# seceq/zkir

Hardware: AMD Instinct MI355X
Metric: trace rows/sec (2^20-cycle fib: execution-trace fill + BabyBear NTT/LDE + Poseidon2 Merkle commitment) (higher is better)
Workload: dtype u32 (Baby Bear, 31-bit modular) / u64 trace words

## Files before the change

### zkir_amd/csrc/host.h

```cpp
#pragma once

#include <sys/mman.h>

#include <atomic>
#include <cstdint>
#include <cstdlib>
#include <cstring>
#include <new>
#include <string>
#include <utility>
#include <vector>

#include "../../include/zkir_amd.h"

#define ZKIR_DEFAULT_TILE_ROWS 1024u

namespace zkir {

struct Status {
  int code = ZKIR_OK;
  std::string msg;
  bool ok() const { return code == ZKIR_OK; }
};

// ... 130 lines not shown
  void* d_block = nullptr;
  const uint32_t* d_tape = nullptr; const uint32_t* h_tape = nullptr;
  const uint64_t* d_side = nullptr;
  const uint64_t* d_prefix = nullptr;
  uint64_t n_words = 0, n_hcells = 0, n_calls = 0;
  HashWitness() = default;
  HashWitness(const HashWitness&) = delete;
  HashWitness& operator=(const HashWitness&) = delete;
  ~HashWitness();
};
int memcheck_device_hash(const zkir_trace_columns* trace, uint64_t n_real, const uint8_t* blob, size_t blob_len, const zkir_hash_out* outs, uint64_t n_outs, uint64_t* mem_old,
                         uint32_t* mem_told, std::vector<uint64_t>& cell_addr, std::vector<uint64_t>& cell_bytes, std::vector<uint32_t>& cell_time, HashWitness& hw, HostPin& pin,
                         void* hip_stream);

struct LdeTables {
  int log_n;
  const uint32_t* tw_inv;
  const uint32_t* tw_fwd;
  const uint32_t* g_lo;
  const uint32_t* g_hi;
  const uint32_t* small_inv;
  const uint32_t* small_fwd;
  int log_blowup = 1;
};
void lde_run(const LdeTables& t, uint32_t* in, uint32_t n_blocks, uint32_t* out, void* hip_stream);
bool strided_variant_run(const LdeTables& t, uint32_t* data, uint32_t n_blocks, int variant, bool dit, void* hip_stream);
bool lde_run_fused01(const LdeTables& t, const zkir_trace_columns* trace, uint64_t n_real, uint32_t* in, uint32_t n_blocks, uint32_t* out, void* hip_stream);
}
```

### zkir_amd/csrc/ntt.hip

```cpp
#include <hip/hip_runtime.h>

#include <atomic>
#include <cstdlib>
#include <mutex>
#include <type_traits>

#include "../../include/zkir_amd.h"
#include "../../include/zkir_amd_experimental.h"
#include "babybear.h"
#include "host.h"

namespace {

constexpr int NT = 256;
__device__ __forceinline__ uint32_t bitrev(uint32_t x, int bits) { return bits == 0 ? 0u : __brev(x) >> (32 - bits); }

template <int K, int N, class F>
__device__ __forceinline__ void static_for(F&& f) {
  if constexpr (K < N) { f(std::integral_constant<int, K>{}); static_for<K + 1, N>(f); }
}

using u32x4 = uint32_t __attribute__((ext_vector_type(4)));
__device__ __forceinline__ u32x4 ld4(const uint4* p) { return *reinterpret_cast<const u32x4*>(p); }
__device__ __forceinline__ void st4(uint4* p, u32x4 v) { *reinterpret_cast<u32x4*>(p) = v; }
// ... 52 lines not shown
  if (blk == 0 && half == 0) {
    const uint64_t pcv = q.t.pc[src];
    r.x = (uint32_t)((q.t.cycle[src] + (i - src)) % bb::P); r.y = (uint32_t)(pcv & 0xFFFFF); r.z = (uint32_t)((pcv >> 20) & 0xFFFFF); r.w = (uint32_t)(pcv >> 40);
  } else if (blk == 0) {
    const uint32_t w = q.t.instruction[src];
    r.x = w & 0x7F; r.y = (w >> 7) & 0xF; r.z = (w >> 11) & 0xF; r.w = (w >> 15) & 0xF;
  } else {
    auto limbs = [&](int g, uint32_t out[3]) {
      const uint64_t o = (uint64_t)g * q.t.reg_stride + src;
      const uint64_t v = q.t.registers[o];
      const int bits = q.t.reg_state[o] ? 30 : 20;
      const uint64_t mask = (1ull << bits) - 1;
      out[0] = (uint32_t)(v & mask); out[1] = (uint32_t)((v >> bits) & mask); out[2] = (uint32_t)(v >> (2 * bits));
    };
    uint32_t a[3], b[3];
    if (half == 0) { limbs(1, a); r.x = q.t.instruction[src] >> 19; r.y = a[0]; r.z = a[1]; r.w = a[2]; }
    else { limbs(2, a); limbs(3, b); r.x = a[0]; r.y = a[1]; r.z = a[2]; r.w = b[0]; }
  }
  return r;
}

template <bool DIT, int R, int C, int NTH, bool FUSED = false>
__global__ __launch_bounds__(NTH) void ntt_strided_r4_kernel(uint4* __restrict__ data, uint64_t blk_u4, uint32_t tiles_per_block, uint32_t total, int L, int s0,
                                                              const uint32_t* __restrict__ tw, const uint32_t* __restrict__ small, int log_small, uint32_t j4_m, int canon, TraceSrc01 fsrc = TraceSrc01{}) {
  constexpr int B = 2 * R;
  constexpr uint32_t POS = 1u << (B + C), QUADS = POS / 4, CMASK = (1u << C) - 1, PLANE = POS + 4;
  constexpr uint32_t MOVES = 2 * POS / NTH;
  static_assert(QUADS % NTH == 0 && NTH % (1 << C) == 0 && (2 * POS) % NTH == 0, "tile / thread geometry");
  extern __shared__ uint4 lds4[];
  const uint32_t n = 1u << L;
  const uint32_t stride_mid = DIT ? (1u << s0) : (n >> (s0 + B));
  const uint32_t lo_tiles = stride_mid >> C;
  auto geometry = [&](uint32_t w, uint4*& x, uint32_t& base, uint32_t& lo0, uint32_t& hi) {
    const uint32_t tile = w % tiles_per_block;
    x = data + (uint64_t)(w / tiles_per_block) * blk_u4;
    hi = tile / lo_tiles;
    lo0 = (tile % lo_tiles) << C;
    base = (DIT ? (hi << (s0 + B)) : hi * (n >> s0)) + lo0;
  };
  static_assert(QUADS == NTH, "one quad per lane and round");
  u32x4 pre[MOVES];
  uint4* x; uint32_t base, lo0, hi;
  uint32_t w = blockIdx.x;
  if (w >= total) return;
  uint32_t sm[R];
#pragma unroll
  for (int r = 0; r < R; r++) {
    const int b = 2 * r;
    const uint32_t qq = threadIdx.x >> C;
    if (!DIT) sm[r] = small[bitrev(qq >> (B - 2 - b), b) << (log_small - (b + 2))];
    else sm[r] = small[(qq & ((1u << b) - 1)) << (log_small - (b + 2))];
  }
  const bool unit = s0 == 0;
  uint32_t tf_next[R] = {};
  auto tile_factors = [&](uint32_t hi_t) {
    if (DIT || unit) return;
    const uint32_t e = bitrev(hi_t, s0);
#pragma unroll
    for (int r = 0; r < R; r++) tf_next[r] = tw[e << (L - s0 - 2 * r - 2)];
  };
  geometry(w, x, base, lo0, hi);
  static_for<0, (int)MOVES>([&](auto kc) {
    constexpr uint32_t k = decltype(kc)::value;
    const uint32_t e = threadIdx.x + k * NTH, row = e >> (C + 1), wv = e & ((2u << C) - 1);
    if constexpr (FUSED) pre[k] = trace_quad01(fsrc, w / tiles_per_block, wv & 1, (uint64_t)base + (uint64_t)row * stride_mid + (wv >> 1));
    else pre[k] = ld4(&x[((uint64_t)base + (uint64_t)row * stride_mid) * 2 + wv]);
  });
  uint32_t tw_cur = 0;
  if (DIT) tw_cur = tw[(lo0 + (threadIdx.x & CMASK)) << (L - s0 - B)];
  tile_factors(hi);
  for (;;) {
    static_for<0, (int)MOVES>([&](auto kc) {
      constexpr uint32_t k = decltype(kc)::value;
      const uint32_t e = threadIdx.x + k * NTH, row = e >> (C + 1), wv = e & ((2u << C) - 1);
      st4(&lds4[(wv & 1) * PLANE + ((row << C) | (wv >> 1))], pre[k]);
    });
    uint32_t tp[R];
    if (DIT) {
      uint32_t u = tw_cur;
#pragma unroll
      for (int r = R - 1; r >= 0; r--) { tp[r] = u; u = bb::mont_mul(u, u); u = bb::mont_mul(u, u); }
    } else {
#pragma unroll
      for (int r = 0; r < R; r++) tp[r] = tf_next[r];
    }
    __syncthreads();
    const uint32_t wn = w + gridDim.x;
    uint4* xn = x; uint32_t base_n = base, lo0_n = lo0, hi_n = hi;
    if (wn < total) {
      geometry(wn, xn, base_n, lo0_n, hi_n);
      static_for<0, (int)MOVES>([&](auto kc) {
        constexpr uint32_t k = decltype(kc)::value;
        const uint32_t e = threadIdx.x + k * NTH, row = e >> (C + 1), wv = e & ((2u << C) - 1);
        if constexpr (FUSED) pre[k] = trace_quad01(fsrc, wn / tiles_per_block, wv & 1, (uint64_t)base_n + (uint64_t)row * stride_mid + (wv >> 1));
        else pre[k] = ld4(&xn[((uint64_t)base_n + (uint64_t)row * stride_mid) * 2 + wv]);
      });
      if (DIT) tw_cur = tw[(lo0_n + (threadIdx.x & CMASK)) << (L - s0 - B)];
      tile_factors(hi_n);
    }
#pragma unroll
    for (int r = 0; r < R; r++) {
      const int b = 2 * r;
#pragma unroll
      for (uint32_t k = 0; k < QUADS / NTH; k++) {
        uint32_t q = threadIdx.x + k * NTH;
        asm volatile("" : "+v"(q));
        const uint32_t lo_l = q & CMASK, qq = q >> C;
        uint4* pl0 = lds4; uint4* pl1 = lds4 + PLANE;
        if constexpr (!DIT) {
          const int lg = B - 2 - b;
          const uint32_t h2 = 1u << lg, mid_lo = qq & (h2 - 1), mid_hi = qq >> lg;
          const uint32_t i0 = ((((mid_hi << (lg + 2)) | mid_lo)) << C) | lo_l, d = h2 << C;
          WTw w1, w2, w2i;
          ct_twiddles(sm[r], tp[r], unit, j4_m, w1, w2, w2i);
          uint4 x0 = pl0[i0], x1 = pl0[i0 + d], x2 = pl0[i0 + 2 * d], x3 = pl0[i0 + 3 * d];
          ct4w4(x0, x1, x2, x3, w1, w2, w2i);
          pl0[i0] = x0; pl0[i0 + d] = x1; pl0[i0 + 2 * d] = x2; pl0[i0 + 3 * d] = x3;
          __builtin_amdgcn_sched_barrier(0);
          uint4 y0 = pl1[i0], y1 = pl1[i0 + d], y2 = pl1[i0 + 2 * d], y3 = pl1[i0 + 3 * d];
          ct4w4(y0, y1, y2, y3, w1, w2, w2i);
          pl1[i0] = y0; pl1[i0 + d] = y1; pl1[i0 + 2 * d] = y2; pl1[i0 + 3 * d] = y3;
        } else {
// ... 1 lines not shown
          const uint32_t i0 = ((((mid_hi << (b + 2)) | mid_lo)) << C) | lo_l, d = dm << C;
          const WTw w2 = wtw(bb::mont_mul_centred(tp[r], sm[r]));
          const uint32_t w2u = bb::wcanon(w2.w);
          const WTw w1 = wtw(bb::mont_mul_centred(w2u, w2u)), w2i = wtw(bb::mont_mul_centred(w2u, j4_m));
          uint4 x0 = pl0[i0], x1 = pl0[i0 + d], x2 = pl0[i0 + 2 * d], x3 = pl0[i0 + 3 * d];
          dit4w4(x0, x1, x2, x3, w1, w2, w2i);
          pl0[i0] = x0; pl0[i0 + d] = x1; pl0[i0 + 2 * d] = x2; pl0[i0 + 3 * d] = x3;
          __builtin_amdgcn_sched_barrier(0);
          uint4 y0 = pl1[i0], y1 = pl1[i0 + d], y2 = pl1[i0 + 2 * d], y3 = pl1[i0 + 3 * d];
          dit4w4(y0, y1, y2, y3, w1, w2, w2i);
          pl1[i0] = y0; pl1[i0 + d] = y1; pl1[i0 + 2 * d] = y2; pl1[i0 + 3 * d] = y3;
        }
      }
      const bool wave_local = !DIT ? (r + 1 < R && B - 2 - b <= 6 - C) : (r + 1 < R && b + 2 <= 6 - C);
      if (wave_local) wave_sync_lds(); else __syncthreads();
    }
#pragma unroll
    for (uint32_t k = 0; k < MOVES; k++) {
      const uint32_t e = threadIdx.x + k * NTH, row = e >> (C + 1), wv = e & ((2u << C) - 1);
      uint4 v = lds4[(wv & 1) * PLANE + ((row << C) | (wv >> 1))];
      if (DIT && canon) v = canon4(v);
      x[((uint64_t)base + (uint64_t)row * stride_mid) * 2 + wv] = v;
    }
    if (wn >= total) break;
    w = wn; x = xn; base = base_n; lo0 = lo0_n; hi = hi_n;
  }
}

template <bool DIT, int S>
__global__ __launch_bounds__(NT) void ntt_reg_kernel(uint4* __restrict__ data, uint64_t blk_u4, int L, int s0, const uint32_t* __restrict__ tw, uint32_t r4_m, uint32_t r8_m,
                                                       uint32_t r8_3_m, int canon) {
  constexpr int E = 1 << S;
  const uint32_t n = 1u << L;
  uint4* x = data + (uint64_t)blockIdx.y * blk_u4;
  const uint64_t item = (uint64_t)blockIdx.x * NT + threadIdx.x;
  if (item >= ((uint64_t)n >> S) * 2) return;
  const uint32_t t = (uint32_t)(item >> 1), h = (uint32_t)(item & 1);
  const uint32_t d = DIT ? (1u << s0) : (n >> (s0 + S));
  const uint32_t hi = t / d, lo = t % d;
  const uint64_t base = ((uint64_t)hi * d * E + lo) * 2 + h;
  uint4 v[E];
#pragma unroll
  for (int k = 0; k < E; k++) v[k] = x[base + (uint64_t)k * d * 2];
  if (!DIT) {
    const uint32_t Tf = tw[bitrev(hi, s0) << (L - s0 - S)];
    const uint32_t Tm = bb::mont_mul(Tf, Tf);
// ... 22 lines not shown
    }
    if (canon) {
#pragma unroll
      for (int k = 0; k < E; k++) v[k] = canon4(v[k]);
    }
  }
#pragma unroll
  for (int k = 0; k < E; k++) x[base + (uint64_t)k * d * 2] = v[k];
}

inline unsigned cu_count() {
  static std::mutex mu;
  static unsigned cached[64] = {};
  int dev = 0;
  if (hipGetDevice(&dev) != hipSuccess || dev < 0 || dev >= 64) return 256u;
  std::lock_guard<std::mutex> lk(mu);
  if (!cached[dev]) { hipDeviceProp_t p; cached[dev] = hipGetDeviceProperties(&p, dev) == hipSuccess && p.multiProcessorCount > 0 ? (unsigned)p.multiProcessorCount : 256u; }
  return cached[dev];
}
inline int persist() { static const int v = getenv("ZKIR_NTT_PERSIST") ? atoi(getenv("ZKIR_NTT_PERSIST")) : 1; return v; }

template <bool DIT, int R, int C, int NTH, bool FUSED = false>
void launch_strided_r4(uint32_t* data, uint64_t n, uint32_t n_blocks, int L, int s0, const uint32_t* tw, const uint32_t* small, int log_small, uint32_t j4_m, hipStream_t s,
                       const TraceSrc01* fsrc = nullptr, int canon = 0) {
  constexpr size_t lds = 16u * 2 * ((1u << (2 * R + C)) + 4);
  auto k = ntt_strided_r4_kernel<DIT, R, C, NTH, FUSED>;
  static std::atomic<uint64_t> attr_done{0};
  int dev = 0; (void)hipGetDevice(&dev);
  const uint64_t bit = 1ull << (dev & 63);
  if (!(attr_done.load(std::memory_order_relaxed) & bit)) { (void)hipFuncSetAttribute(reinterpret_cast<const void*>(k), hipFuncAttributeMaxDynamicSharedMemorySize, (int)lds); attr_done.fetch_or(bit); }
  const uint32_t tiles = (uint32_t)(n >> (2 * R + C)), total = tiles * n_blocks;
  const unsigned per_cu = (unsigned)((160u << 10) / lds) > 0 ? (unsigned)((160u << 10) / lds) : 1u;
  unsigned grid = persist() ? cu_count() * (per_cu > 8 ? 8 : per_cu) : total;
  if (grid > total) grid = total;
  hipLaunchKernelGGL(k, dim3(grid), dim3(NTH), lds, s, (uint4*)data, 2 * n, tiles, total, L, s0, tw, small, log_small, j4_m, canon, fsrc ? *fsrc : TraceSrc01{});
}

inline int strided_c() { static const int c = getenv("ZKIR_NTT_C") ? atoi(getenv("ZKIR_NTT_C")) : 2; return c; }

template <bool DIT>
void run_strided_stages(uint32_t* data, uint64_t n, uint32_t n_blocks, int L, int s0, int stages, const uint32_t* tw, const uint32_t* small, int log_small, uint32_t j4_m,
                        uint32_t r8_m, uint32_t r8_3_m, hipStream_t s) {
  while (stages > 0) {
    int take;
    if (stages >= 10 && stages != 11) take = 10;
    else if (stages == 11) take = 8;
    else if (stages == 9) take = 6;
    else if (stages == 7) take = 4;
    else if (stages == 5) take = 3;
    else take = stages;
    const int canon = DIT && take == stages;
    switch (take) {
      case 10:
        if (strided_c() == 2) launch_strided_r4<DIT, 5, 2, 1024>(data, n, n_blocks, L, s0, tw, small, log_small, j4_m, s, nullptr, canon);
        else launch_strided_r4<DIT, 5, 1, 512>(data, n, n_blocks, L, s0, tw, small, log_small, j4_m, s, nullptr, canon);
        break;
      case 8: launch_strided_r4<DIT, 4, 3, 512>(data, n, n_blocks, L, s0, tw, small, log_small, j4_m, s, nullptr, canon); break;
      case 6: launch_strided_r4<DIT, 3, 4, 256>(data, n, n_blocks, L, s0, tw, small, log_small, j4_m, s, nullptr, canon); break;
      case 4: launch_strided_r4<DIT, 2, 5, 128>(data, n, n_blocks, L, s0, tw, small, log_small, j4_m, s, nullptr, canon); break;
      case 3:
        hipLaunchKernelGGL((ntt_reg_kernel<DIT, 3>), dim3((unsigned)(((n >> 3) * 2 + NT - 1) / NT), n_blocks), dim3(NT), 0, s, (uint4*)data, 2 * n, L, s0, tw, j4_m, r8_m, r8_3_m, canon);
        break;
      case 2:
        hipLaunchKernelGGL((ntt_reg_kernel<DIT, 2>), dim3((unsigned)(((n >> 2) * 2 + NT - 1) / NT), n_blocks), dim3(NT), 0, s, (uint4*)data, 2 * n, L, s0, tw, j4_m, r8_m, r8_3_m, canon);
        break;
      default:
        hipLaunchKernelGGL(ntt_stage_kernel<DIT>, dim3((unsigned)((n + NT - 1) / NT), n_blocks), dim3(NT), 0, s, (uint4*)data, 2 * n, L, s0, tw, canon);
        break;
    }
    s0 += take; stages -= take;
  }
}

__global__ __launch_bounds__(NT) void lde_small_kernel(const uint32_t* __restrict__ in, uint32_t* __restrict__ out, int L, const uint32_t* __restrict__ small_inv,
                                                        const uint32_t* __restrict__ small_fwd, const uint32_t* __restrict__ g_lo, const uint32_t* __restrict__ g_hi) {
  extern __shared__ uint32_t lds[];
  const uint32_t n = 1u << L;
  const uint32_t* x = in + (uint64_t)blockIdx.x * n * 8;
  uint32_t* y = out + (uint64_t)blockIdx.x * 2 * n * 8;
  for (int c = 0; c < 8; c++) {
    for (uint32_t e = threadIdx.x; e < n; e += NT) lds[e] = x[(uint64_t)e * 8 + c];
    __syncthreads();
    for (int b = 0; b < L; b++) {
      const int hb = L - 1 - b;
      const uint32_t half = 1u << hb;
      for (uint32_t q = threadIdx.x; q < (n >> 1); q += NT) {
        const uint32_t r_lo = q & (half - 1), r_hi = q >> hb;
        const uint32_t ia = (r_hi << (hb + 1)) | r_lo, ib = ia + half;
        const uint32_t a = lds[ia], bv = lds[ib];
        lds[ia] = bb::add(a, bv); lds[ib] = bb::mont_mul(bb::sub(a, bv), small_inv[r_lo << b]);
      }
      __syncthreads();
    }
    uint32_t v[2];
// ... 1 lines not shown
    for (uint32_t e = threadIdx.x; e < n; e += NT) { const uint32_t k = bitrev(e, L); v[cnt++] = bb::mont_mul(bb::mont_mul(lds[e], g_lo[k & 1023]), g_hi[k >> 10]); }
    __syncthreads();
    cnt = 0;
    for (uint32_t e = threadIdx.x; e < n; e += NT) { lds[2 * e] = v[cnt]; lds[2 * e + 1] = v[cnt]; cnt++; }
    __syncthreads();
    for (int s = 1; s <= L; s++) {
      const uint32_t half = 1u << s;
      for (uint32_t q = threadIdx.x; q < n; q += NT) {
        const uint32_t r_lo = q & (half - 1), r_hi = q >> s;
        const uint32_t ia = (r_hi << (s + 1)) | r_lo, ib = ia + half;
        const uint32_t a = lds[ia], t = bb::mont_mul(lds[ib], small_fwd[r_lo << (L - s)]);
        lds[ia] = bb::add(a, t); lds[ib] = bb::sub(a, t);
      }
      __syncthreads();
    }
    for (uint32_t e = threadIdx.x; e < 2 * n; e += NT) y[(uint64_t)e * 8 + c] = lds[e];
    __syncthreads();
  }
}

constexpr int MID_NT = 512;
__global__ __launch_bounds__(MID_NT) __attribute__((amdgpu_waves_per_eu(4, 4))) void lde_middle_r4_kernel(const uint4* __restrict__ in, uint4* __restrict__ out, uint32_t chunks_per_block, uint32_t total, int L,
                                                                const uint32_t* __restrict__ tw_inv, const uint32_t* __restrict__ small_inv, const uint32_t* __restrict__ small_fwd,
                                                                const uint32_t* __restrict__ g_lo, const uint32_t* __restrict__ g_hi, uint32_t j4_inv_m, uint32_t j4_fwd_m, int canon) {
  constexpr int Bm = 10;
  constexpr uint32_t APL = 1024;
  __shared__ uint4 A[2 * APL];
  __shared__ uint4 Bf[2048];
  const uint32_t n = 1u << L, t = threadIdx.x;
  uint32_t w = blockIdx.x;
  if (w >= total) return;
  uint32_t tw_i[5], tw_f[5];
#pragma unroll
  for (int r = 0; r < 5; r++) {
    const int lg = 8 - 2 * r;
    tw_i[r] = small_inv[bitrev((t & 255) >> lg, 2 * r) << lg];
    const int sft = 2 * r + 1;
    tw_f[r] = small_fwd[(t & ((1u << sft) - 1)) << (Bm - sft - 1)];
  }
  u32x4 pre[4];
  uint32_t cf_next[5];
  uint32_t glo[4], ghi[4];
  auto fetch = [&](uint32_t ww) {
    const uint4* x = in + ((uint64_t)(ww / chunks_per_block) * n + ((uint64_t)(ww % chunks_per_block) << Bm)) * 2;
#pragma unroll
    for (int k = 0; k < 4; k++) pre[k] = ld4(&x[t + k * MID_NT]);
    const uint32_t p0 = ((ww % chunks_per_block) << Bm) + 4 * (t & 255);
#pragma unroll
    for (int i = 0; i < 4; i++) { const uint32_t k = bitrev(p0 + i, L); glo[i] = g_lo[k & 1023]; ghi[i] = g_hi[k >> 10]; }
    const uint32_t ce = bitrev(ww % chunks_per_block, L - Bm);
#pragma unroll
    for (int r = 0; r < 5; r++) cf_next[r] = tw_inv[ce << (8 - 2 * r)];
  };
  fetch(w);
  for (;;) {
    const uint32_t base = (w % chunks_per_block) << Bm;
    uint4* y = out + (uint64_t)(w / chunks_per_block) * n * 4;
#pragma unroll
    for (int k = 0; k < 4; k++) { const uint32_t e = t + k * MID_NT; st4(&A[(e & 1) * APL + (e >> 1)], pre[k]); }
    uint32_t gs[4];
#pragma unroll
    for (int i = 0; i < 4; i++) gs[i] = bb::mont_mul(glo[i], ghi[i]);
    uint32_t cf[5];
#pragma unroll
    for (int r = 0; r < 5; r++) cf[r] = cf_next[r];
    __syncthreads();
    const uint32_t wn = w + gridDim.x;
    if (wn < total) fetch(wn);
    {
      const uint32_t q = t & 255;
      uint4* a = A + (t >> 8) * APL;
#pragma unroll
      for (int r = 0; r < 5; r++) {
        const int lg = 8 - 2 * r;
        const uint32_t h2 = 1u << lg, lo = q & (h2 - 1), hi = q >> lg;
        const uint32_t i0 = (hi << (lg + 2)) | lo;
        WTw c1, c2, c2i;
        ct_twiddles(tw_i[r], cf[r], false, j4_inv_m, c1, c2, c2i);
        uint4 x0 = a[i0], x1 = a[i0 + h2], x2 = a[i0 + 2 * h2], x3 = a[i0 + 3 * h2];
        ct4w4(x0, x1, x2, x3, c1, c2, c2i);
        if (r == 4) {
          x0 = scale4(x0, gs[0]); x1 = scale4(x1, gs[1]); x2 = scale4(x2, gs[2]); x3 = scale4(x3, gs[3]);
        }
        a[i0] = x0; a[i0 + h2] = x1; a[i0 + 2 * h2] = x2; a[i0 + 3 * h2] = x3;
        if (r >= 1 && r < 4) wave_sync_lds(); else __syncthreads();
      }
    }
#pragma unroll 1
    for (int h = 0; h < 2; h++) {
      const uint4* a = A + h * APL;
// ... 183 lines not shown
  static const uint32_t j4_inv_m = bb::to_mont(bb::inv(bb::root_of_unity(2))), j4_fwd_m = bb::to_mont(bb::root_of_unity(2));
  static const uint32_t r8_fwd = bb::root_of_unity(3), r8_inv = bb::inv(r8_fwd);
  static const uint32_t r8_inv_m = bb::to_mont(r8_inv), r8_inv3_m = bb::to_mont(bb::mul(bb::mul(r8_inv, r8_inv), r8_inv));
  static const uint32_t r8_fwd_m = bb::to_mont(r8_fwd), r8_fwd3_m = bb::to_mont(bb::mul(bb::mul(r8_fwd, r8_fwd), r8_fwd));
  const int LB = t.log_blowup;
  if (LB != 1) {
    if (L < 10) {
      hipLaunchKernelGGL(lde_small_blowup_kernel, dim3(n_blocks), dim3(NT), (4u << (L + LB)), s, in, out, L, LB, t.small_inv, t.small_fwd, t.g_lo, t.g_hi);
      return;
    }
    run_strided_stages<false>(in, N, n_blocks, L, 0, L - 10, t.tw_inv, t.small_inv, 10, j4_inv_m, r8_inv_m, r8_inv3_m, s);
    const uint32_t chunks = N >> 10, total = chunks * n_blocks;
    unsigned grid = persist() ? cu_count() * 2 : total;
    if (grid > total) grid = total;
    auto mid = LB == 2 ? lde_middle_blowup_kernel<2> : lde_middle_blowup_kernel<3>;
    hipLaunchKernelGGL(mid, dim3(grid), dim3(MID_NT), 0, s, (const uint4*)in, (uint4*)out, chunks, total, L, t.tw_inv, t.small_inv, t.small_fwd, t.g_lo, t.g_hi, j4_inv_m, j4_fwd_m, L == 10);
    run_strided_stages<true>(out, (uint64_t)N << LB, n_blocks, L + LB, 10 + LB, L - 10, t.tw_fwd, t.small_fwd, 10 + LB, j4_fwd_m, r8_fwd_m, r8_fwd3_m, s);
    return;
  }
  if (L < 10) {
    hipLaunchKernelGGL(lde_small_kernel, dim3(n_blocks), dim3(NT), (8u << L), s, in, out, L, t.small_inv, t.small_fwd, t.g_lo, t.g_hi);
    return;
  }
  run_strided_stages<false>(in, N, n_blocks, L, 0, L - 10, t.tw_inv, t.small_inv, 10, j4_inv_m, r8_inv_m, r8_inv3_m, s);
  {
    const uint32_t chunks = N >> 10, total = chunks * n_blocks;
    unsigned grid = persist() ? cu_count() * 2 : total;
    if (grid > total) grid = total;
    hipLaunchKernelGGL(lde_middle_r4_kernel, dim3(grid), dim3(MID_NT), 0, s, (const uint4*)in, (uint4*)out, chunks, total, L, t.tw_inv, t.small_inv, t.small_fwd, t.g_lo, t.g_hi,
                       j4_inv_m, j4_fwd_m, L == 10);
  }
  run_strided_stages<true>(out, (uint64_t)2 * N, n_blocks, L + 1, 11, L - 10, t.tw_fwd, t.small_fwd, 11, j4_fwd_m, r8_fwd_m, r8_fwd3_m, s);
}


bool strided_variant_run(const LdeTables& t, uint32_t* data, uint32_t n_blocks, int variant, bool dit, void* stream) {
  hipStream_t s = (hipStream_t)stream;
  const int L = dit ? t.log_n + 1 : t.log_n;
  if (t.log_n < 20) return false;
  const uint64_t n = (uint64_t)1 << L;
  static const uint32_t j4_inv_m = bb::to_mont(bb::inv(bb::root_of_unity(2))), j4_fwd_m = bb::to_mont(bb::root_of_unity(2));
  const uint32_t* tw = dit ? t.tw_fwd : t.tw_inv; const uint32_t* sm = dit ? t.small_fwd : t.small_inv;
  const int ls = dit ? 11 : 10; const uint32_t j4 = dit ? j4_fwd_m : j4_inv_m; const int s0 = dit ? 11 : 0;
#define ZKIR_VARIANT(R, C, NTH) do { if (dit) launch_strided_r4<true, R, C, NTH>(data, n, n_blocks, L, s0, tw, sm, ls, j4, s); else launch_strided_r4<false, R, C, NTH>(data, n, n_blocks, L, s0, tw, sm, ls, j4, s); } while (0)
  switch (variant) {
    case 0: ZKIR_VARIANT(5, 2, 1024); break;
    case 1: ZKIR_VARIANT(5, 1, 512); break;
    case 2: ZKIR_VARIANT(4, 3, 512); break;
    case 3: ZKIR_VARIANT(4, 2, 256); break;
    case 4: ZKIR_VARIANT(3, 4, 256); break;
    default: return false;
  }
#undef ZKIR_VARIANT
  return true;
}

bool lde_run_fused01(const LdeTables& t, const zkir_trace_columns* trace, uint64_t n_real, uint32_t* in, uint32_t n_blocks, uint32_t* out, void* stream) {
  hipStream_t s = (hipStream_t)stream;
  const int L = t.log_n;
  if (L < 20 || L == 21 || n_blocks < 3 || strided_c() != 2) return false;
  const uint32_t N = 1u << L;
  static const uint32_t j4_inv_m = bb::to_mont(bb::inv(bb::root_of_unity(2))), j4_fwd_m = bb::to_mont(bb::root_of_unity(2));
  static const uint32_t r8_fwd = bb::root_of_unity(3), r8_inv = bb::inv(r8_fwd);
  static const uint32_t r8_inv_m = bb::to_mont(r8_inv), r8_inv3_m = bb::to_mont(bb::mul(bb::mul(r8_inv, r8_inv), r8_inv));
  static const uint32_t r8_fwd_m = bb::to_mont(r8_fwd), r8_fwd3_m = bb::to_mont(bb::mul(bb::mul(r8_fwd, r8_fwd), r8_fwd));
  const TraceSrc01 src{*trace, n_real};
  launch_strided_r4<false, 5, 2, 1024, true>(in, N, 2, L, 0, t.tw_inv, t.small_inv, 10, j4_inv_m, s, &src);
  launch_strided_r4<false, 5, 2, 1024>(in + (uint64_t)2 * N * 8, N, n_blocks - 2, L, 0, t.tw_inv, t.small_inv, 10, j4_inv_m, s);
  if (L - 10 > 10) run_strided_stages<false>(in, N, n_blocks, L, 10, L - 20, t.tw_inv, t.small_inv, 10, j4_inv_m, r8_inv_m, r8_inv3_m, s);
  {
    const uint32_t chunks = N >> 10, total = chunks * n_blocks;
    unsigned grid = persist() ? cu_count() * 2 : total;
    if (grid > total) grid = total;
    hipLaunchKernelGGL(lde_middle_r4_kernel, dim3(grid), dim3(MID_NT), 0, s, (const uint4*)in, (uint4*)out, chunks, total, L, t.tw_inv, t.small_inv, t.small_fwd, t.g_lo, t.g_hi,
                       j4_inv_m, j4_fwd_m, L == 10);
  }
  run_strided_stages<true>(out, (uint64_t)2 * N, n_blocks, L + 1, 11, L - 10, t.tw_fwd, t.small_fwd, 11, j4_fwd_m, r8_fwd_m, r8_fwd3_m, s);
  return true;
}

}
```

### zkir_amd/csrc/stark.hip

```cpp
#include <hip/hip_runtime.h>

#include <array>
#include <atomic>
#include <chrono>
#include <cstdio>
#include <cstdlib>
#include <cstddef>
#include <memory>
#include <mutex>
#include <vector>

#include "../../include/zkir_amd.h"
#include "../../include/zkir_amd_experimental.h"
#include "air.h"
#include "babybear.h"
#include "fri_shape.h"
#include "host.h"
#include "hashcall.h"
#include "poseidon2.h"
#include "verify_stages.h"

namespace {

constexpr int NT = 256;
// ... 577 lines not shown
}

__global__ __launch_bounds__(NT) void modmul_peak_kernel(uint32_t* __restrict__ out, uint32_t iters) {
  uint32_t a[8], c[8];
#pragma unroll
  for (int k = 0; k < 8; k++) { a[k] = (threadIdx.x * 2654435761u + blockIdx.x * 40503u + k * 7919u) % bb::P; c[k] = (a[k] * 31u + 7u) % bb::P; }
  for (uint32_t i = 0; i < iters; i++) {
#pragma unroll
    for (int k = 0; k < 8; k++) a[k] = bb::mont_mul_lazy(a[k], c[k]);
  }
  uint32_t r = 0;
#pragma unroll
  for (int k = 0; k < 8; k++) r ^= a[k];
  if (r == 0xFFFFFFFFu && iters == 0xFFFFFFFFu) out[0] = r;
}

constexpr uint32_t SYNC_SLOTS = 1024;
struct SyncRing {
  uint32_t* d_slots = nullptr;
  std::atomic<uint32_t> next{0};
  uint32_t* take() { return d_slots + (next.fetch_add(1, std::memory_order_relaxed) % SYNC_SLOTS); }
};

void launch_tree_levels(const p2::Consts* cp, uint32_t* leaf_digests, uint64_t n_leaves, SyncRing& ring, hipStream_t s) {
  uint32_t* cur = leaf_digests;
  uint64_t m = n_leaves;
  for (; m > (1u << 18); m >>= 1) {
    uint32_t* nxt = cur + 4 * m;
    hipLaunchKernelGGL(compress_kernel, dim3(grid_for(m / 2)), dim3(NT), 0, s, cp, cur, m / 2, nxt);
    cur = nxt;
  }
  if (m > 1) {
    const uint32_t per = m < SUBTREE ? (uint32_t)m : SUBTREE;
    hipLaunchKernelGGL(subtree_kernel, dim3((unsigned)(m / per)), dim3(NT_SUB), 0, s, cp, cur, m, per, ring.take());
  }
}

}

struct zkir_stark_ctx {
  uint32_t log_n = 0, log_blowup = 1;
  uint32_t* d_tw_inv = nullptr;
  uint32_t* d_tw_fwd = nullptr;
  uint32_t* d_g_lo = nullptr;
  uint32_t* d_g_lo_m = nullptr;
  mutable uint32_t* d_inv_xm1 = nullptr;
  uint32_t* d_g_hi = nullptr;
  uint32_t* d_small_inv = nullptr;
  uint32_t* d_small_fwd = nullptr;
  p2::Consts consts;
  p2::Consts* d_p2 = nullptr;
  mutable hipStream_t ov_stream = nullptr; mutable hipEvent_t ov_ev[2] = {nullptr, nullptr}; mutable std::vector<hipEvent_t> ov_group_ev; mutable uint4* d_ov_state = nullptr; mutable size_t ov_state_bytes = 0;
  mutable SyncRing sync;
  mutable std::mutex mu;
  mutable unsigned char* arena = nullptr;
  mutable size_t arena_size = 0, arena_off = 0;
  mutable zkir::HostPin pin;
  mutable const uint32_t* rate_mats[3] = {nullptr, nullptr, nullptr};
  mutable uint32_t rate_widths[3] = {0, 0, 0};
};

namespace {
const char* const BLOWUP2_ONLY = ": the context has log_blowup != 1; the prover's quotient, DEEP and FRI stages (and the experiments built on its LDE) are blow-up 2 — contexts of log_blowup 2 / 3 serve zkir_lde_launch and the zkir_merkle_* calls";
bool blowup2_only(const zkir_stark_ctx* c, const char* who) {
  if (c->log_blowup == 1) return true;
  zkir::set_last_error({ZKIR_ERR_ARGUMENT, std::string(who) + BLOWUP2_ONLY});
  return false;
}
int lde_launch(const zkir_stark_ctx* c, uint32_t* in, uint32_t width, uint32_t* out, bool mont_out, hipStream_t s) {
  const zkir::LdeTables t{(int)c->log_n, c->d_tw_inv, c->d_tw_fwd, mont_out ? c->d_g_lo_m : c->d_g_lo, c->d_g_hi, c->d_small_inv, c->d_small_fwd, (int)c->log_blowup};
  zkir::lde_run(t, in, (width + 7) / 8, out, s);
  return check_launch("lde");
}
int merkle_commit(const zkir_stark_ctx* c, const uint32_t* mat, uint32_t width, uint64_t n_leaves, uint32_t* tree, bool mont_in, hipStream_t s) {
  hipLaunchKernelGGL(leaf_hash_kernel, dim3(grid_for(n_leaves)), dim3(NT), 0, s, c->d_p2, mat, width, n_leaves, mont_in ? bb::from_mont(c->consts.in_scale) : c->consts.in_scale, tree);
  launch_tree_levels(c->d_p2, tree, n_leaves, c->sync, s);
  return check_launch("merkle_commit");
}
int selector_table_ensure(const zkir_stark_ctx* c, hipStream_t s) {
  if (c->d_inv_xm1) return ZKIR_OK;
  const uint64_t M = 1ull << (c->log_n + c->log_blowup);
  uint32_t* t = nullptr;
  if (hipMalloc(&t, (size_t)M * 4) != hipSuccess) { zkir::set_last_error({ZKIR_ERR_DEVICE, "zkir_prove_rate: no device memory for the selector table"}); return ZKIR_ERR_DEVICE; }
  hipLaunchKernelGGL(selector_inverse_kernel, dim3(grid_for((M + 7) / 8)), dim3(NT), 0, s, c->log_n + c->log_blowup, c->d_tw_fwd, t);
  c->d_inv_xm1 = t;
  return check_launch("selector table");
}
}

extern "C" {

uint32_t zkir_main_trace_width(void) { return air::committed_width(false); }
uint32_t zkir_main_trace_width_for(uint32_t deferred) { return air::committed_width((int)deferred); }
// ... 69 lines not shown
  (void)hipEventSynchronize(b);
  float ms = 0;
  (void)hipEventElapsedTime(&ms, a, b);
  (void)hipEventDestroy(a); (void)hipEventDestroy(b); (void)hipFree(d);
  return ms > 0 ? (double)blocks * NT * iters * 8.0 / (ms * 1e-3) : 0.0;
}

int zkir_stark_ctx_create(uint32_t log_n, uint32_t log_blowup, zkir_stark_ctx** out) {
  if (!out || log_n < 1 || log_n > 26 || log_blowup < 1 || log_blowup > 3 || log_n + log_blowup > 27) {
    zkir::set_last_error({ZKIR_ERR_ARGUMENT, "zkir_stark_ctx_create: need 1 <= log_n <= 26, log_blowup in {1, 2, 3} and log_n + log_blowup <= 27 (the field's two-adicity)"});
    return ZKIR_ERR_ARGUMENT;
  }
  *out = nullptr;
  zkir_stark_ctx* c = new zkir_stark_ctx();
  c->log_n = log_n; c->log_blowup = log_blowup;
  const uint32_t N = 1u << log_n;
  const uint32_t n_inv = N >= 2 ? N / 2 : 1, n_hi = (N >> 10) + 1;
  const uint32_t n_fwd = N << (log_blowup - 1);
  p2::generate(c->consts);
  hipError_t e = hipMalloc((void**)&c->d_p2, sizeof(p2::Consts));
  if (e == hipSuccess) e = hipMemcpy(c->d_p2, &c->consts, sizeof(p2::Consts), hipMemcpyHostToDevice);
  if (e == hipSuccess) e = hipMalloc(&c->sync.d_slots, SYNC_SLOTS * sizeof(uint32_t));
  if (e == hipSuccess) e = hipMemset(c->sync.d_slots, 0, SYNC_SLOTS * sizeof(uint32_t));
  if (e == hipSuccess) e = hipMalloc(&c->d_tw_inv, (size_t)n_inv * 4);
  if (e == hipSuccess) e = hipMalloc(&c->d_tw_fwd, (size_t)n_fwd * 4);
  if (e == hipSuccess) e = hipMalloc(&c->d_g_lo, 1024 * 4);
  if (e == hipSuccess) e = hipMalloc(&c->d_g_hi, (size_t)n_hi * 4);
  if (e == hipSuccess) e = hipMalloc(&c->d_g_lo_m, 1024 * 4);
  if (e == hipSuccess && log_blowup == 1) e = hipMalloc(&c->d_inv_xm1, (size_t)2 * N * 4);
  const int Bm = log_n < 10 ? (int)log_n : 10;
  const uint32_t n_si = Bm >= 1 ? (1u << (Bm - 1)) : 1, n_sf = 1u << (Bm + log_blowup - 1);
  if (e == hipSuccess) e = hipMalloc(&c->d_small_inv, (size_t)n_si * 4);
  if (e == hipSuccess) e = hipMalloc(&c->d_small_fwd, (size_t)n_sf * 4);
  if (e != hipSuccess) { zkir::set_last_error({ZKIR_ERR_DEVICE, std::string("zkir_stark_ctx_create: ") + hipGetErrorString(e)}); zkir_stark_ctx_free(c); return ZKIR_ERR_DEVICE; }
  const uint32_t wN = bb::root_of_unity(log_n), wM = bb::root_of_unity(log_n + log_blowup);
  hipLaunchKernelGGL(powers_kernel, dim3(grid_for(n_inv)), dim3(NT), 0, 0, bb::inv(wN), bb::R1, c->d_tw_inv, n_inv);
  hipLaunchKernelGGL(powers_kernel, dim3(grid_for(n_fwd)), dim3(NT), 0, 0, wM, bb::R1, c->d_tw_fwd, n_fwd);
  hipLaunchKernelGGL(powers_kernel, dim3(4), dim3(NT), 0, 0, bb::GEN, bb::to_mont(bb::inv(N % bb::P)), c->d_g_lo, 1024u);
  hipLaunchKernelGGL(powers_kernel, dim3(4), dim3(NT), 0, 0, bb::GEN, bb::to_mont(bb::to_mont(bb::inv(N % bb::P))), c->d_g_lo_m, 1024u);
  hipLaunchKernelGGL(powers_kernel, dim3(grid_for(n_hi)), dim3(NT), 0, 0, bb::pow(bb::GEN, 1024), bb::R1, c->d_g_hi, n_hi);
  if (log_blowup == 1) hipLaunchKernelGGL(selector_inverse_kernel, dim3(grid_for((2ull * N + 7) / 8)), dim3(NT), 0, 0, log_n + 1, c->d_tw_fwd, c->d_inv_xm1);
  hipLaunchKernelGGL(powers_kernel, dim3(grid_for(n_si)), dim3(NT), 0, 0, bb::inv(bb::root_of_unity(Bm)), bb::R1, c->d_small_inv, n_si);
  hipLaunchKernelGGL(powers_kernel, dim3(grid_for(n_sf)), dim3(NT), 0, 0, bb::root_of_unity(Bm + log_blowup), bb::R1, c->d_small_fwd, n_sf);
  if (hipDeviceSynchronize() != hipSuccess || check_launch("stark ctx tables") != ZKIR_OK) { zkir_stark_ctx_free(c); return ZKIR_ERR_DEVICE; }
  *out = c;
  return ZKIR_OK;
}

void zkir_stark_ctx_free(zkir_stark_ctx* c) {
  if (!c) return;
  (void)hipFree(c->d_tw_inv); (void)hipFree(c->d_tw_fwd); (void)hipFree(c->d_g_lo); (void)hipFree(c->d_g_hi); (void)hipFree(c->d_g_lo_m); (void)hipFree(c->d_inv_xm1);
  (void)hipFree(c->d_small_inv); (void)hipFree(c->d_small_fwd); (void)hipFree(c->d_p2); (void)hipFree(c->sync.d_slots);
  if (c->ov_stream) (void)hipStreamDestroy(c->ov_stream);
  for (hipEvent_t e : c->ov_ev) if (e) (void)hipEventDestroy(e);
  for (hipEvent_t e : c->ov_group_ev) (void)hipEventDestroy(e);
  (void)hipFree(c->d_ov_state);
  if (c->arena) (void)hipFree(c->arena);
  delete c;
}

uint32_t zkir_stark_ctx_log_blowup(const zkir_stark_ctx* c) { return c ? c->log_blowup : 0; }

uint32_t zkir_padded_log_n(uint64_t n_real) { uint32_t k = 3; while (((uint64_t)1 << k) < n_real) k++; return k; }

int zkir_main_trace_launch(const zkir_trace_columns* trace, uint64_t n_real, uint32_t deferred, uint32_t* out, void* stream) {
  if (!trace || !out || n_real == 0 || deferred > 1) { zkir::set_last_error({ZKIR_ERR_ARGUMENT, "zkir_main_trace_launch: null argument, empty trace, or a mode other than 0 / 1 (mode 2: zkir_main_trace_io_launch)"}); return ZKIR_ERR_ARGUMENT; }
  const uint64_t N = (uint64_t)1 << zkir_padded_log_n(n_real);
  if (deferred) hipLaunchKernelGGL(main_trace_kernel<1>, dim3(grid_for(N)), dim3(NT), 0, (hipStream_t)stream, *trace, n_real, N, out, IoRowArgs{});
  else hipLaunchKernelGGL(main_trace_kernel<0>, dim3(grid_for(N)), dim3(NT), 0, (hipStream_t)stream, *trace, n_real, N, out, IoRowArgs{});
  return check_launch("main_trace");
}
int zkir_main_trace_io_launch(const zkir_trace_columns* trace, uint64_t n_real, const zkir_io_args* io, uint32_t* scratch, uint32_t* out, void* stream) {
  if (!trace || !out || !io || !scratch || n_real == 0 || (!io->inputs && io->n_inputs)) { zkir::set_last_error({ZKIR_ERR_ARGUMENT, "zkir_main_trace_io_launch: null argument or empty trace"}); return ZKIR_ERR_ARGUMENT; }
  hipStream_t s = (hipStream_t)stream;
  const uint64_t N = (uint64_t)1 << zkir_padded_log_n(n_real);
// ... 158 lines not shown
```

Baseline: 190.7 million.

## Skip NTT/LDE work for all-zero column blocks via device zero flags

The first strided inverse-NTT pass now ORs the tile data it loads and, per column block, records an epoch-tagged flag when any nonzero value appears. The middle LDE kernel and the forward strided passes read these flags with a ballot. For blocks never flagged, the middle kernel writes zeros to the output and the forward kernels skip the butterfly work. Zero columns in the padded trace therefore cost far less compute. The price is an extra block-wide reduction in the first pass, a ring of flag slots on the device, and reliance on the first pass covering every tile of a block before the later kernels read the flags.

```diff
diff --git a/zkir_amd/csrc/host.h b/zkir_amd/csrc/host.h
--- a/zkir_amd/csrc/host.h
+++ b/zkir_amd/csrc/host.h
@@ -176,7 +176,10 @@
   const uint32_t* small_inv;
   const uint32_t* small_fwd;
   int log_blowup = 1;
+  uint32_t* zero_slot = nullptr;
+  uint32_t zero_epoch = 0;
 };
+constexpr uint32_t ZERO_FLAG_BLOCKS = 64;
 void lde_run(const LdeTables& t, uint32_t* in, uint32_t n_blocks, uint32_t* out, void* hip_stream);
 bool strided_variant_run(const LdeTables& t, uint32_t* data, uint32_t n_blocks, int variant, bool dit, void* hip_stream);
 bool lde_run_fused01(const LdeTables& t, const zkir_trace_columns* trace, uint64_t n_real, uint32_t* in, uint32_t n_blocks, uint32_t* out, void* hip_stream);
diff --git a/zkir_amd/csrc/ntt.hip b/zkir_amd/csrc/ntt.hip
--- a/zkir_amd/csrc/ntt.hip
+++ b/zkir_amd/csrc/ntt.hip
@@ -98,7 +98,8 @@
 
 template <bool DIT, int R, int C, int NTH, bool FUSED = false>
 __global__ __launch_bounds__(NTH) void ntt_strided_r4_kernel(uint4* __restrict__ data, uint64_t blk_u4, uint32_t tiles_per_block, uint32_t total, int L, int s0,
-                                                              const uint32_t* __restrict__ tw, const uint32_t* __restrict__ small, int log_small, uint32_t j4_m, int canon, TraceSrc01 fsrc = TraceSrc01{}) {
+                                                              const uint32_t* __restrict__ tw, const uint32_t* __restrict__ small, int log_small, uint32_t j4_m, int canon, TraceSrc01 fsrc = TraceSrc01{},
+                                                              uint32_t* zflags = nullptr, uint32_t epoch = 0, int produce = 0) {
   constexpr int B = 2 * R;
   constexpr uint32_t POS = 1u << (B + C), QUADS = POS / 4, CMASK = (1u << C) - 1, PLANE = POS + 4;
   constexpr uint32_t MOVES = 2 * POS / NTH;
@@ -117,7 +118,10 @@
   static_assert(QUADS == NTH, "one quad per lane and round");
   u32x4 pre[MOVES];
   uint4* x; uint32_t base, lo0, hi;
-  uint32_t w = blockIdx.x;
+  uint64_t live = ~0ull;
+  if (zflags && !produce) { const uint32_t l = threadIdx.x & 63; live = __ballot(l < total / tiles_per_block && zflags[l] == epoch); }
+  auto next_live = [&](uint32_t ww) { while (ww < total && !((live >> (ww / tiles_per_block)) & 1)) ww += gridDim.x; return ww; };
+  uint32_t w = next_live(blockIdx.x);
   if (w >= total) return;
   uint32_t sm[R];
 #pragma unroll
@@ -146,10 +150,12 @@
   if (DIT) tw_cur = tw[(lo0 + (threadIdx.x & CMASK)) << (L - s0 - B)];
   tile_factors(hi);
   for (;;) {
+    uint32_t nz = 0;
     static_for<0, (int)MOVES>([&](auto kc) {
       constexpr uint32_t k = decltype(kc)::value;
       const uint32_t e = threadIdx.x + k * NTH, row = e >> (C + 1), wv = e & ((2u << C) - 1);
       st4(&lds4[(wv & 1) * PLANE + ((row << C) | (wv >> 1))], pre[k]);
+      if (produce) nz |= (pre[k].x | pre[k].y) | (pre[k].z | pre[k].w);
     });
     uint32_t tp[R];
     if (DIT) {
@@ -160,8 +166,14 @@
 #pragma unroll
       for (int r = 0; r < R; r++) tp[r] = tf_next[r];
     }
-    __syncthreads();
-    const uint32_t wn = w + gridDim.x;
+    bool dense = true;
+    if (produce) {
+      dense = __syncthreads_or(nz != 0) != 0;
+      if (dense && threadIdx.x == 0) zflags[w / tiles_per_block] = epoch;
+    } else {
+      __syncthreads();
+    }
+    const uint32_t wn = next_live(w + gridDim.x);
     uint4* xn = x; uint32_t base_n = base, lo0_n = lo0, hi_n = hi;
     if (wn < total) {
       geometry(wn, xn, base_n, lo0_n, hi_n);
@@ -174,6 +186,7 @@
       if (DIT) tw_cur = tw[(lo0_n + (threadIdx.x & CMASK)) << (L - s0 - B)];
       tile_factors(hi_n);
     }
+    if (dense) {
 #pragma unroll
     for (int r = 0; r < R; r++) {
       const int b = 2 * r;
@@ -221,6 +234,7 @@
       if (DIT && canon) v = canon4(v);
       x[((uint64_t)base + (uint64_t)row * stride_mid) * 2 + wv] = v;
     }
+    }
     if (wn >= total) break;
     w = wn; x = xn; base = base_n; lo0 = lo0_n; hi = hi_n;
   }
@@ -289,7 +303,7 @@
 
 template <bool DIT, int R, int C, int NTH, bool FUSED = false>
 void launch_strided_r4(uint32_t* data, uint64_t n, uint32_t n_blocks, int L, int s0, const uint32_t* tw, const uint32_t* small, int log_small, uint32_t j4_m, hipStream_t s,
-                       const TraceSrc01* fsrc = nullptr, int canon = 0) {
+                       const TraceSrc01* fsrc = nullptr, int canon = 0, uint32_t* zflags = nullptr, uint32_t epoch = 0, int produce = 0) {
   constexpr size_t lds = 16u * 2 * ((1u << (2 * R + C)) + 4);
   auto k = ntt_strided_r4_kernel<DIT, R, C, NTH, FUSED>;
   static std::atomic<uint64_t> attr_done{0};
@@ -300,14 +314,15 @@
   const unsigned per_cu = (unsigned)((160u << 10) / lds) > 0 ? (unsigned)((160u << 10) / lds) : 1u;
   unsigned grid = persist() ? cu_count() * (per_cu > 8 ? 8 : per_cu) : total;
   if (grid > total) grid = total;
-  hipLaunchKernelGGL(k, dim3(grid), dim3(NTH), lds, s, (uint4*)data, 2 * n, tiles, total, L, s0, tw, small, log_small, j4_m, canon, fsrc ? *fsrc : TraceSrc01{});
+  hipLaunchKernelGGL(k, dim3(grid), dim3(NTH), lds, s, (uint4*)data, 2 * n, tiles, total, L, s0, tw, small, log_small, j4_m, canon, fsrc ? *fsrc : TraceSrc01{}, zflags, epoch, produce);
 }
 
 inline int strided_c() { static const int c = getenv("ZKIR_NTT_C") ? atoi(getenv("ZKIR_NTT_C")) : 2; return c; }
 
 template <bool DIT>
-void run_strided_stages(uint32_t* data, uint64_t n, uint32_t n_blocks, int L, int s0, int stages, const uint32_t* tw, const uint32_t* small, int log_small, uint32_t j4_m,
-                        uint32_t r8_m, uint32_t r8_3_m, hipStream_t s) {
+uint32_t* run_strided_stages(uint32_t* data, uint64_t n, uint32_t n_blocks, int L, int s0, int stages, const uint32_t* tw, const uint32_t* small, int log_small, uint32_t j4_m,
+                             uint32_t r8_m, uint32_t r8_3_m, hipStream_t s, uint32_t* zflags = nullptr, uint32_t epoch = 0, bool produce = false) {
+  bool first = true;
   while (stages > 0) {
     int take;
     if (stages >= 10 && stages != 11) take = 10;
@@ -317,14 +332,17 @@
     else if (stages == 5) take = 3;
     else take = stages;
     const int canon = DIT && take == stages;
+    int pr = 0;
+    if (produce && first) { if (take >= 4) pr = 1; else zflags = nullptr; }
+    first = false;
     switch (take) {
       case 10:
-        if (strided_c() == 2) launch_strided_r4<DIT, 5, 2, 1024>(data, n, n_blocks, L, s0, tw, small, log_small, j4_m, s, nullptr, canon);
-        else launch_strided_r4<DIT, 5, 1, 512>(data, n, n_blocks, L, s0, tw, small, log_small, j4_m, s, nullptr, canon);
+        if (strided_c() == 2) launch_strided_r4<DIT, 5, 2, 1024>(data, n, n_blocks, L, s0, tw, small, log_small, j4_m, s, nullptr, canon, zflags, epoch, pr);
+        else launch_strided_r4<DIT, 5, 1, 512>(data, n, n_blocks, L, s0, tw, small, log_small, j4_m, s, nullptr, canon, zflags, epoch, pr);
         break;
-      case 8: launch_strided_r4<DIT, 4, 3, 512>(data, n, n_blocks, L, s0, tw, small, log_small, j4_m, s, nullptr, canon); break;
-      case 6: launch_strided_r4<DIT, 3, 4, 256>(data, n, n_blocks, L, s0, tw, small, log_small, j4_m, s, nullptr, canon); break;
-      case 4: launch_strided_r4<DIT, 2, 5, 128>(data, n, n_blocks, L, s0, tw, small, log_small, j4_m, s, nullptr, canon); break;
+      case 8: launch_strided_r4<DIT, 4, 3, 512>(data, n, n_blocks, L, s0, tw, small, log_small, j4_m, s, nullptr, canon, zflags, epoch, pr); break;
+      case 6: launch_strided_r4<DIT, 3, 4, 256>(data, n, n_blocks, L, s0, tw, small, log_small, j4_m, s, nullptr, canon, zflags, epoch, pr); break;
+      case 4: launch_strided_r4<DIT, 2, 5, 128>(data, n, n_blocks, L, s0, tw, small, log_small, j4_m, s, nullptr, canon, zflags, epoch, pr); break;
       case 3:
         hipLaunchKernelGGL((ntt_reg_kernel<DIT, 3>), dim3((unsigned)(((n >> 3) * 2 + NT - 1) / NT), n_blocks), dim3(NT), 0, s, (uint4*)data, 2 * n, L, s0, tw, j4_m, r8_m, r8_3_m, canon);
         break;
@@ -337,6 +355,7 @@
     }
     s0 += take; stages -= take;
   }
+  return zflags;
 }
 
 __global__ __launch_bounds__(NT) void lde_small_kernel(const uint32_t* __restrict__ in, uint32_t* __restrict__ out, int L, const uint32_t* __restrict__ small_inv,
@@ -384,13 +403,24 @@
 constexpr int MID_NT = 512;
 __global__ __launch_bounds__(MID_NT) __attribute__((amdgpu_waves_per_eu(4, 4))) void lde_middle_r4_kernel(const uint4* __restrict__ in, uint4* __restrict__ out, uint32_t chunks_per_block, uint32_t total, int L,
                                                                 const uint32_t* __restrict__ tw_inv, const uint32_t* __restrict__ small_inv, const uint32_t* __restrict__ small_fwd,
-                                                                const uint32_t* __restrict__ g_lo, const uint32_t* __restrict__ g_hi, uint32_t j4_inv_m, uint32_t j4_fwd_m, int canon) {
+                                                                const uint32_t* __restrict__ g_lo, const uint32_t* __restrict__ g_hi, uint32_t j4_inv_m, uint32_t j4_fwd_m, int canon,
+                                                                const uint32_t* __restrict__ zflags, uint32_t epoch) {
   constexpr int Bm = 10;
   constexpr uint32_t APL = 1024;
   __shared__ uint4 A[2 * APL];
   __shared__ uint4 Bf[2048];
   const uint32_t n = 1u << L, t = threadIdx.x;
-  uint32_t w = blockIdx.x;
+  uint64_t live = ~0ull;
+  if (zflags) { const uint32_t l = t & 63; live = __ballot(l < total / chunks_per_block && zflags[l] == epoch); }
+  auto next_live = [&](uint32_t ww) {
+    for (; ww < total && !((live >> (ww / chunks_per_block)) & 1); ww += gridDim.x) {
+      uint4* yz = out + (uint64_t)(ww / chunks_per_block) * n * 4 + ((uint64_t)(ww % chunks_per_block) << (Bm + 2));
+#pragma unroll
+      for (int k = 0; k < 4; k++) { const uint32_t e = t + k * MID_NT; yz[2 * e] = make_uint4(0, 0, 0, 0); yz[2 * e + 1] = make_uint4(0, 0, 0, 0); }
+    }
+    return ww;
+  };
+  uint32_t w = next_live(blockIdx.x);
   if (w >= total) return;
   uint32_t tw_i[5], tw_f[5];
 #pragma unroll
@@ -427,7 +457,7 @@
 #pragma unroll
     for (int r = 0; r < 5; r++) cf[r] = cf_next[r];
     __syncthreads();
-    const uint32_t wn = w + gridDim.x;
+    const uint32_t wn = next_live(w + gridDim.x);
     if (wn < total) fetch(wn);
     {
       const uint32_t q = t & 255;
@@ -657,15 +687,16 @@
     hipLaunchKernelGGL(lde_small_kernel, dim3(n_blocks), dim3(NT), (8u << L), s, in, out, L, t.small_inv, t.small_fwd, t.g_lo, t.g_hi);
     return;
   }
-  run_strided_stages<false>(in, N, n_blocks, L, 0, L - 10, t.tw_inv, t.small_inv, 10, j4_inv_m, r8_inv_m, r8_inv3_m, s);
+  uint32_t* zf = t.zero_slot && t.zero_epoch && n_blocks <= ZERO_FLAG_BLOCKS ? t.zero_slot : nullptr;
+  zf = run_strided_stages<false>(in, N, n_blocks, L, 0, L - 10, t.tw_inv, t.small_inv, 10, j4_inv_m, r8_inv_m, r8_inv3_m, s, zf, t.zero_epoch, zf != nullptr);
   {
     const uint32_t chunks = N >> 10, total = chunks * n_blocks;
     unsigned grid = persist() ? cu_count() * 2 : total;
     if (grid > total) grid = total;
     hipLaunchKernelGGL(lde_middle_r4_kernel, dim3(grid), dim3(MID_NT), 0, s, (const uint4*)in, (uint4*)out, chunks, total, L, t.tw_inv, t.small_inv, t.small_fwd, t.g_lo, t.g_hi,
-                       j4_inv_m, j4_fwd_m, L == 10);
-  }
-  run_strided_stages<true>(out, (uint64_t)2 * N, n_blocks, L + 1, 11, L - 10, t.tw_fwd, t.small_fwd, 11, j4_fwd_m, r8_fwd_m, r8_fwd3_m, s);
+                       j4_inv_m, j4_fwd_m, L == 10, (const uint32_t*)zf, t.zero_epoch);
+  }
+  run_strided_stages<true>(out, (uint64_t)2 * N, n_blocks, L + 1, 11, L - 10, t.tw_fwd, t.small_fwd, 11, j4_fwd_m, r8_fwd_m, r8_fwd3_m, s, zf, t.zero_epoch);
 }
 
 
@@ -708,7 +739,7 @@
     unsigned grid = persist() ? cu_count() * 2 : total;
     if (grid > total) grid = total;
     hipLaunchKernelGGL(lde_middle_r4_kernel, dim3(grid), dim3(MID_NT), 0, s, (const uint4*)in, (uint4*)out, chunks, total, L, t.tw_inv, t.small_inv, t.small_fwd, t.g_lo, t.g_hi,
-                       j4_inv_m, j4_fwd_m, L == 10);
+                       j4_inv_m, j4_fwd_m, L == 10, nullptr, 0u);
   }
   run_strided_stages<true>(out, (uint64_t)2 * N, n_blocks, L + 1, 11, L - 10, t.tw_fwd, t.small_fwd, 11, j4_fwd_m, r8_fwd_m, r8_fwd3_m, s);
   return true;
diff --git a/zkir_amd/csrc/stark.hip b/zkir_amd/csrc/stark.hip
--- a/zkir_amd/csrc/stark.hip
+++ b/zkir_amd/csrc/stark.hip
@@ -623,6 +623,17 @@
   uint32_t* take() { return d_slots + (next.fetch_add(1, std::memory_order_relaxed) % SYNC_SLOTS); }
 };
 
+constexpr uint32_t ZERO_SLOTS = 1024;
+struct ZeroFlagRing {
+  uint32_t* d_words = nullptr;
+  std::atomic<uint32_t> next{0};
+  void take(uint32_t*& slot, uint32_t& epoch) {
+    uint32_t e = next.fetch_add(1, std::memory_order_relaxed) + 1;
+    if (e == 0) e = next.fetch_add(1, std::memory_order_relaxed) + 1;
+    slot = d_words + (size_t)(e % ZERO_SLOTS) * zkir::ZERO_FLAG_BLOCKS; epoch = e;
+  }
+};
+
 void launch_tree_levels(const p2::Consts* cp, uint32_t* leaf_digests, uint64_t n_leaves, SyncRing& ring, hipStream_t s) {
   uint32_t* cur = leaf_digests;
   uint64_t m = n_leaves;
@@ -653,6 +664,7 @@
   p2::Consts* d_p2 = nullptr;
   mutable hipStream_t ov_stream = nullptr; mutable hipEvent_t ov_ev[2] = {nullptr, nullptr}; mutable std::vector<hipEvent_t> ov_group_ev; mutable uint4* d_ov_state = nullptr; mutable size_t ov_state_bytes = 0;
   mutable SyncRing sync;
+  mutable ZeroFlagRing zero;
   mutable std::mutex mu;
   mutable unsigned char* arena = nullptr;
   mutable size_t arena_size = 0, arena_off = 0;
@@ -669,7 +681,8 @@
   return false;
 }
 int lde_launch(const zkir_stark_ctx* c, uint32_t* in, uint32_t width, uint32_t* out, bool mont_out, hipStream_t s) {
-  const zkir::LdeTables t{(int)c->log_n, c->d_tw_inv, c->d_tw_fwd, mont_out ? c->d_g_lo_m : c->d_g_lo, c->d_g_hi, c->d_small_inv, c->d_small_fwd, (int)c->log_blowup};
+  zkir::LdeTables t{(int)c->log_n, c->d_tw_inv, c->d_tw_fwd, mont_out ? c->d_g_lo_m : c->d_g_lo, c->d_g_hi, c->d_small_inv, c->d_small_fwd, (int)c->log_blowup};
+  if (c->log_blowup == 1 && c->log_n >= 14) c->zero.take(t.zero_slot, t.zero_epoch);
   zkir::lde_run(t, in, (width + 7) / 8, out, s);
   return check_launch("lde");
 }
@@ -785,6 +798,8 @@
   if (e == hipSuccess) e = hipMemcpy(c->d_p2, &c->consts, sizeof(p2::Consts), hipMemcpyHostToDevice);
   if (e == hipSuccess) e = hipMalloc(&c->sync.d_slots, SYNC_SLOTS * sizeof(uint32_t));
   if (e == hipSuccess) e = hipMemset(c->sync.d_slots, 0, SYNC_SLOTS * sizeof(uint32_t));
+  if (e == hipSuccess) e = hipMalloc(&c->zero.d_words, (size_t)ZERO_SLOTS * zkir::ZERO_FLAG_BLOCKS * sizeof(uint32_t));
+  if (e == hipSuccess) e = hipMemset(c->zero.d_words, 0, (size_t)ZERO_SLOTS * zkir::ZERO_FLAG_BLOCKS * sizeof(uint32_t));
   if (e == hipSuccess) e = hipMalloc(&c->d_tw_inv, (size_t)n_inv * 4);
   if (e == hipSuccess) e = hipMalloc(&c->d_tw_fwd, (size_t)n_fwd * 4);
   if (e == hipSuccess) e = hipMalloc(&c->d_g_lo, 1024 * 4);
@@ -813,7 +828,7 @@
 void zkir_stark_ctx_free(zkir_stark_ctx* c) {
   if (!c) return;
   (void)hipFree(c->d_tw_inv); (void)hipFree(c->d_tw_fwd); (void)hipFree(c->d_g_lo); (void)hipFree(c->d_g_hi); (void)hipFree(c->d_g_lo_m); (void)hipFree(c->d_inv_xm1);
-  (void)hipFree(c->d_small_inv); (void)hipFree(c->d_small_fwd); (void)hipFree(c->d_p2); (void)hipFree(c->sync.d_slots);
+  (void)hipFree(c->d_small_inv); (void)hipFree(c->d_small_fwd); (void)hipFree(c->d_p2); (void)hipFree(c->sync.d_slots); (void)hipFree(c->zero.d_words);
   if (c->ov_stream) (void)hipStreamDestroy(c->ov_stream);
   for (hipEvent_t e : c->ov_ev) if (e) (void)hipEventDestroy(e);
   for (hipEvent_t e : c->ov_group_ev) (void)hipEventDestroy(e);
```

New measurement: 202.5 million (median of 6 runs). 1.06x the previous value.
